# wenyuqing/panacea

Hardware: AMD Instinct MI355X
Metric: denoising steps/s (6-view x 8-frame 256x512) (higher is better)
Workload: dtype f16; 1 GPU; BASELINE config 3: Panacea+ stage-2 UNet+ControlNet, CFG 2 x 8 frames, 6 views, latent 32x384, hint 256x3072, Euler/LegacyDDPM 50-step schedule; precision=precise: split(stream,gn_stt,ff_out,stem,gn_head,gnt)+e4m3-lo, parallelism=single, graph=False, streams=2, hoisted_step_invariants=False, fused_step_tail=True

## Files before the change

### include/panacea_hip.h

```cpp
#ifndef PANACEA_HIP_H
#define PANACEA_HIP_H

#include <stdint.h>

#ifdef __cplusplus
extern "C" {
#endif

#define PNC_OK 0
#define PNC_EINVAL (-1)
#define PNC_EALIGN (-2)
#define PNC_EABI (-3)

const char* pnc_version(void);
#define PNC_ABI_VERSION 8
int pnc_abi_version(void);
const char* pnc_build_digest(void);

enum {
    PNC_OPT_GEMM_TAIL_SPLIT = 0,
    PNC_OPT_GEMM_TILE = 1,
    PNC_OPT_ATTN_VARIANT = 2,
    PNC_OPT_ATTN_DMA = 3,
    PNC_OPT_GEMM_FUSE_LN = 4,
// ... 124 lines not shown
#define PNC_SMALLM_MAX_SEGS 64
int pnc_linear_smallm_segments(const float* a, int lda, const void* W, const float* bias, float* out, int M,
                               int m0, int Mtot, int N, int K, const int32_t* seg_start, int nseg, int silu_in,
                               int silu_out, void* stream);
int pnc_linear_smallm_segments_split(const float* a, int lda, const void* W, const void* W_lo, const float* bias, float* out,
                                     int M, int m0, int Mtot, int N, int K, const int32_t* seg_start, int nseg, int silu_in,
                                     int silu_out, void* stream);
int pnc_timestep_embedding(const int64_t* t, int F, int dim, const float* freqs,
                           float* out, void* stream);
int pnc_timestep_embedding_f32(const float* t, int F, int dim, const float* freqs,
                               float* out, void* stream);
int pnc_nchw_to_tokens_f16(const float* a, int C1, const float* a_scale, int a_frames, const float* b, int C2,
                           int F, int Npix, int Cpad, void* out16, void* out16_lo, void* stream);
int pnc_cfg_euler_step(const float* eps_tok, int ld, int T, int Npix, int C, int cfg, float scale,
                       const float* x, const float* c_out, const float* sigma, const float* sigma_next, float* x_next,
                       void* stream);
enum {
    PNC_SAMPLER_HEUN1 = 0, PNC_SAMPLER_HEUN2 = 1, PNC_SAMPLER_EULER_A = 2, PNC_SAMPLER_DPM2S_1 = 3, PNC_SAMPLER_DPM2S_2 = 4,
    PNC_SAMPLER_DPM2M = 5, PNC_SAMPLER_LMS = 6
};
typedef struct PncSamplerStepParams {
    int32_t struct_bytes;
    int32_t mode;
    const float* eps_tok;
    int32_t ld, T, Npix, C;
    int32_t cfg;
    float scale;
    const float* x;
    const float* c_out;
    const float* x0;
    const float* aux;
    const float* hist[4];
    int32_t n_hist;
    float s_noise;
    const float* noise;
    const float* v[6];
    float* out;
    float* out_aux;
} PncSamplerStepParams;
int pnc_cfg_sampler_step(const PncSamplerStepParams* p, void* stream);
int pnc_cfg_euler_step_skip(const float* eps_tok, int ld, int T, int Npix, int C, int cfg, float scale,
                            const float* x, const float* c_skip, const float* c_out, const float* sigma,
                            const float* sigma_next, float* x_next, void* stream);
int pnc_cfg_sampler_step_skip(const PncSamplerStepParams* p, const float* c_skip, void* stream);
int pnc_tokens_to_nchw_f32(const float* x, int ld, int F, int Npix, int C,
                           float* out, void* stream);
int pnc_concat_add(const float* a, int C1, const float* s, const float* c, int C2,
                   int64_t M, float* out32, void* out16, void* out16_lo, int lo_fmt, void* stream);
int pnc_concat_add_stats(const float* a, int C1, const float* s, const float* c, int C2, int F, int Npix, int pix_per_chunk,
                         float* out32, void* out16, void* out16_lo, int lo_fmt, float* partial, void* stream);
int pnc_add_f32(const float* x, const float* a, int64_t n, float* y32, void* y16, void* y16_lo, int lo_fmt,
                void* stream);
int pnc_cast_f16(const float* x, int64_t n, void* y16, void* y16_lo, int lo_fmt, void* stream);

int pnc_range_monitor_collect(unsigned int* out, void* stream);

#define PNC_STATS_WORDS 36
int pnc_operand_stats_f16(const void* hi, const void* lo, int lo_fmt, int64_t rows, int cols, int64_t ld,
                          unsigned long long* rec, void* stream);

int pnc_softmax_rows_f16(const float* s, int64_t lds, int M, int N, float scale, int causal, int n_valid,
                         void* p16, int64_t ldp, void* stream);

int pnc_attn_frame_f16(const void* q, int64_t ldq, const void* k, int64_t ldk,
                       const void* vt, int64_t ldvt, int64_t vt_fstride,
                       void* o, int64_t ldo, int F, int N, int C, float scale, void* stream);

int pnc_attn_frame_split_f16(const void* q, const void* q_lo, int64_t ldq, const void* k, const void* k_lo, int64_t ldk,
                             const void* v, const void* v_lo, int64_t ldv, void* o, void* o_lo, int64_t ldo,
                             int F, int N, int C, float scale, void* stream);

int pnc_attn_text_split_f16(const void* q, const void* q_lo, int64_t ldq, const void* k, const void* k_lo, int64_t ldk,
                            const void* v, const void* v_lo, int64_t ldv, void* o, void* o_lo, int64_t ldo,
                            int groups, int heads, int Lp, int kv_valid, float scale, void* stream);

int pnc_u8_to_tokens_f16(const uint8_t* src, const float* lut, int F, int Npix, int C, int Cpad,
                         void* out16, void* out16_lo, void* stream);
int pnc_tokens_to_u8(const float* x, int ld, int64_t M, int C, uint8_t* out, void* stream);

#ifdef __cplusplus
}
#endif
#endif
```

### panacea_amd/csrc/misc.hip

```cpp
#include "common.h"
#include <atomic>

namespace {

constexpr int SM_MAXM = 16;

__global__ __launch_bounds__(256) void linear_smallm_kernel(const float* __restrict__ a, int lda,
                                                            const half_t* __restrict__ W,
                                                            const half_t* __restrict__ W_lo,
                                                            const float* __restrict__ bias,
                                                            float* __restrict__ out, int ldo, int M, int N,
                                                            int K, int silu_in, int silu_out) {
    const int lane = threadIdx.x & 63;
    const int n = blockIdx.x * 4 + (threadIdx.x >> 6);
    if (n >= N) return;
    float acc[SM_MAXM];
#pragma unroll
    for (int m = 0; m < SM_MAXM; ++m) acc[m] = 0.0f;
    for (int k0 = lane * 8; k0 < K; k0 += 64 * 8) {
        const half8v w = *reinterpret_cast<const half8v*>(W + (int64_t)n * K + k0);
        float wf[8];
#pragma unroll
        for (int e = 0; e < 8; ++e) wf[e] = (float)w[e];
        if (W_lo) {
// ... 140 lines not shown
                                                             int Npix, int C, float* __restrict__ out) {
    const int64_t i = (int64_t)blockIdx.x * 256 + threadIdx.x;
    if (i >= (int64_t)F * Npix) return;
    const int64_t f = i / Npix, pix = i - f * Npix;
    for (int c = 0; c < C; ++c) out[(f * C + c) * Npix + pix] = x[i * ld + c];
}

__global__ __launch_bounds__(256) void concat_add_kernel(const float* __restrict__ a, int C1,
                                                         const float* __restrict__ s,
                                                         const float* __restrict__ c, int C2, int64_t M,
                                                         float* __restrict__ out32, half_t* __restrict__ out16,
                                                         void* __restrict__ out16_lo, int lo_fmt) {
    const int CT = C1 + C2, V = CT >> 2;
    const int64_t i = (int64_t)blockIdx.x * 256 + threadIdx.x;
    if (i >= M * V) return;
    const int64_t m = i / V;
    const int ch = (int)(i - m * V) * 4;
    f32x4 v;
    if (ch < C1) {
        v = *reinterpret_cast<const f32x4*>(a + m * C1 + ch);
    } else {
        const int c2 = ch - C1;
        v = *reinterpret_cast<const f32x4*>(s + m * C2 + c2);
        if (c) {
            const f32x4 w = *reinterpret_cast<const f32x4*>(c + m * C2 + c2);
            v += w;
        }
    }
    if (out32) *reinterpret_cast<f32x4*>(out32 + m * CT + ch) = v;
    if (out16) {
        half4v h = {(half_t)v[0], (half_t)v[1], (half_t)v[2], (half_t)v[3]};
        *reinterpret_cast<half4v*>(out16 + m * CT + ch) = h;
        if (out16_lo) {
            const float o[4] = {v[0], v[1], v[2], v[3]};
            store_lo4(out16_lo, lo_fmt, m * CT + ch, o, h);
        }
    }
}

__global__ __launch_bounds__(256) void add_kernel(const float* __restrict__ x, const float* __restrict__ a,
                                                  int64_t n4, float* __restrict__ y32, half_t* __restrict__ y16,
                                                  void* __restrict__ y16_lo, int lo_fmt) {
    const int64_t i = (int64_t)blockIdx.x * 256 + threadIdx.x;
    if (i >= n4) return;
    f32x4 v = *reinterpret_cast<const f32x4*>(x + i * 4);
    if (a) { const f32x4 w = *reinterpret_cast<const f32x4*>(a + i * 4); v += w; }
    if (y32) *reinterpret_cast<f32x4*>(y32 + i * 4) = v;
    if (y16) {
        half4v h = {(half_t)v[0], (half_t)v[1], (half_t)v[2], (half_t)v[3]};
        *reinterpret_cast<half4v*>(y16 + i * 4) = h;
        if (y16_lo) {
            const float o[4] = {v[0], v[1], v[2], v[3]};
            store_lo4(y16_lo, lo_fmt, i * 4, o, h);
        }
    }
}

template <bool SKIP>
__device__ __forceinline__ float guided_denoised(float xv, float eu, float ec, float co, float cs, int cfg, float scale) {
#pragma clang fp contract(off)
    const float xs = SKIP ? xv * cs : xv;
    const float pc = ec * co;
    float D = pc + xs;
    if (cfg) {
        const float pu = eu * co;
        const float du = pu + xs;
        const float g = scale * (D - du);
        D = du + g;
    }
    return D;
}

template <bool SKIP>
__global__ __launch_bounds__(256) void cfg_sampler_step_kernel(const PncSamplerStepParams p, const float* __restrict__ c_skip) {
#pragma clang fp contract(off)
    const int64_t i = (int64_t)blockIdx.x * 256 + threadIdx.x;
    if (i >= (int64_t)p.T * p.Npix) return;
    const int64_t t = i / p.Npix, pix = i - t * p.Npix;
    const float co = p.c_out[t];
    const float cs = SKIP ? c_skip[t] : 1.0f;
    const float v0 = p.v[0] ? p.v[0][t] : 0.f, v1 = p.v[1] ? p.v[1][t] : 0.f, v2 = p.v[2] ? p.v[2][t] : 0.f;
    const float v3 = p.v[3] ? p.v[3][t] : 0.f, v4 = p.v[4] ? p.v[4][t] : 0.f;
    const float* eu = p.eps_tok + i * p.ld;
    const float* ec = p.eps_tok + ((int64_t)(p.cfg ? p.T : 0) * p.Npix + i) * p.ld;
    for (int c = 0; c < p.C; ++c) {
        const int64_t o = (t * p.C + c) * p.Npix + pix;
        const float xv = p.x[o];
        const float D = guided_denoised<SKIP>(xv, eu[c], ec[c], co, cs, p.cfg, p.scale);
        float y;
        switch (p.mode) {
        case PNC_SAMPLER_HEUN1: {
            const float d = (xv - D) / v0;
            const float dt = v1 - v0;
            const float stp = dt * d;
            y = xv + stp;
            if (p.out_aux) p.out_aux[o] = d;
            break;
        }
        case PNC_SAMPLER_HEUN2: {
            const float d_new = (xv - D) / v1;
            const float sum = p.aux[o] + d_new;
            const float dp = sum / 2.0f;
            const float dt = v1 - v0;
            const float stp = dp * dt;
            const float xc = p.x0[o] + stp;
            y = v1 > 0.f ? xc : xv;
// ... 178 lines not shown
        segs.start[i] = seg_start[i];
    }
    return launch_1d(linear_smallm_seg_kernel, (int64_t)(N / SEG_NC) * 64, stream, a, lda, f16p(W), f16p(W_lo), bias, out, M, m0, Mtot,
                     N, K, silu_in, silu_out, segs);
}

template <typename TS>
static int timestep_embedding(const TS* t, int F, int dim, const float* freqs, float* out, void* stream) {
    if (!t || !out || !freqs || F < 1 || dim < 2) return PNC_EINVAL;
    return launch_1d(timestep_embedding_kernel<TS>, F * (dim / 2), stream, t, F, dim, freqs, out);
}

extern "C" int pnc_timestep_embedding(const int64_t* t, int F, int dim, const float* freqs,
                                      float* out, void* stream) {
    return timestep_embedding(t, F, dim, freqs, out, stream);
}

extern "C" int pnc_timestep_embedding_f32(const float* t, int F, int dim, const float* freqs,
                                          float* out, void* stream) {
    return timestep_embedding(t, F, dim, freqs, out, stream);
}

extern "C" int pnc_nchw_to_tokens_f16(const float* a, int C1, const float* a_scale, int a_frames, const float* b, int C2,
                                      int F, int Npix, int Cpad, void* out16, void* out16_lo, void* stream) {
    if (!a || !out16 || F < 1 || Npix < 1 || C1 < 1 || C2 < 0 || (C2 > 0 && !b)) return PNC_EINVAL;
    if (a_frames < 1 || a_frames > F) return PNC_EINVAL;
    if (Cpad % 8 || Cpad < C1 + C2) return PNC_EINVAL;
    if (((uintptr_t)out16 | (uintptr_t)out16_lo) & 15) return PNC_EALIGN;
    return launch_1d(nchw_to_tokens_kernel, (int64_t)F * Npix, stream, a, C1, a_scale, a_frames, b, C2, F, Npix, Cpad, f16p(out16),
                     f16p(out16_lo));
}

extern "C" int pnc_tokens_to_nchw_f32(const float* x, int ld, int F, int Npix, int C,
                                      float* out, void* stream) {
    if (!x || !out || F < 1 || Npix < 1 || C < 1 || ld < C) return PNC_EINVAL;
    return launch_1d(tokens_to_nchw_kernel, (int64_t)F * Npix, stream, x, ld, F, Npix, C, out);
}

extern "C" int pnc_concat_add(const float* a, int C1, const float* s, const float* c, int C2,
                              int64_t M, float* out32, void* out16, void* out16_lo, int lo_fmt, void* stream) {
    if (!a || !s || M < 1 || C1 % 4 || C2 % 4 || C1 < 4 || C2 < 4) return PNC_EINVAL;
    if (lo_fmt != PNC_LO_F16 && lo_fmt != PNC_LO_E4M3) return PNC_EINVAL;
    if ((!out32 && !out16) || (out16_lo && !out16)) return PNC_EINVAL;
    return launch_1d(concat_add_kernel, M * ((C1 + C2) / 4), stream, a, C1, s, c, C2, M, out32, f16p(out16), out16_lo, lo_fmt);
}

extern "C" int pnc_add_f32(const float* x, const float* a, int64_t n, float* y32, void* y16, void* y16_lo, int lo_fmt,
                           void* stream) {
    if (!x || n < 4 || n % 4 || (!y32 && !y16) || (y16_lo && !y16)) return PNC_EINVAL;
    if (lo_fmt != PNC_LO_F16 && lo_fmt != PNC_LO_E4M3) return PNC_EINVAL;
    return launch_1d(add_kernel, n / 4, stream, x, a, n / 4, y32, f16p(y16), y16_lo, lo_fmt);
}

__global__ __launch_bounds__(256) void softmax_rows_kernel(const float* __restrict__ s, int64_t lds, int N, float scale,
                                                           int causal, int n_valid,
                                                           half_t* __restrict__ p, int64_t ldp) {
    __shared__ float red[8];
    const int tid = threadIdx.x, lane = tid & 63, wave = tid >> 6;
    const float* row = s + (int64_t)blockIdx.x * lds;
    half_t* prow = p + (int64_t)blockIdx.x * ldp;
    const int nv = N >> 2;
    const int lim = causal ? min(n_valid, (int)blockIdx.x + 1) : n_valid;
    f32x4 v[16];
    float m = -3.0e38f;
#pragma unroll
    for (int j = 0; j < 16; ++j) {
        const int c = tid + j * 256;
        if (c < nv) {
            v[j] = *reinterpret_cast<const f32x4*>(row + c * 4);
#pragma unroll
            for (int e = 0; e < 4; ++e) v[j][e] = (c * 4 + e < lim) ? v[j][e] : -3.0e38f;
            m = fmaxf(fmaxf(fmaxf(v[j][0], v[j][1]), fmaxf(v[j][2], v[j][3])), m);
        }
    }
#pragma unroll
    for (int o = 32; o > 0; o >>= 1) m = fmaxf(m, __shfl_xor(m, o, 64));
    if (lane == 0) red[wave] = m;
    __syncthreads();
    m = fmaxf(fmaxf(red[0], red[1]), fmaxf(red[2], red[3]));
    const float sc = scale * 1.44269504088896340736f;
    const float off = m * sc;
    float sum = 0.0f;
#pragma unroll
    for (int j = 0; j < 16; ++j) {
        const int c = tid + j * 256;
        if (c < nv) {
#pragma unroll
            for (int e = 0; e < 4; ++e) {
                const float pe = __builtin_amdgcn_exp2f(fmaf(v[j][e], sc, -off));
                v[j][e] = (c * 4 + e < lim) ? pe : 0.0f;
                sum += v[j][e];
            }
        }
    }
    sum = wave_sum(sum);
    if (lane == 0) red[4 + wave] = sum;
    __syncthreads();
    const float inv = 1.0f / (((red[4] + red[5]) + red[6]) + red[7]);
#pragma unroll
    for (int j = 0; j < 16; ++j) {
        const int c = tid + j * 256;
        if (c < nv) {
            half4v h;
#pragma unroll
            for (int e = 0; e < 4; ++e) h[e] = (half_t)(v[j][e] * inv);
            *reinterpret_cast<half4v*>(prow + c * 4) = h;
// ... 32 lines not shown
```

### panacea_amd/engine.py

```python
from __future__ import annotations

import contextlib
import dataclasses
import math
import os
from dataclasses import dataclass
from typing import Callable, Dict, List, NamedTuple, Optional

import torch

from . import hip as _hip
from .shard import FrameShard, ViewShard

_BACKEND = _hip


def backend():
    return _BACKEND


@contextlib.contextmanager
def use_backend(be):
    global _BACKEND
    old, _BACKEND = _BACKEND, be
# ... 213 lines not shown
            raise ValueError(f"at most {TEXT_PAD} context tokens are supported, got {n}")
        if D % 8:
            raise ValueError("context_dim must be a multiple of 8")
        self.n_text = n
        if self.prec.ctx:
            c32 = torch.zeros((B, TEXT_PAD, D), device=self.device, dtype=torch.float32)
            c32[:, :n] = context.to(device=self.device, dtype=torch.float32)
            self.ctx16 = self.operand((B * TEXT_PAD, D), "ctx")
            self.be.cast_f16(c32, c32.numel(), *self.ctx16)
            return
        c = torch.zeros((B, TEXT_PAD, D), device=self.device, dtype=torch.float16)
        c[:, :n] = context.to(device=self.device, dtype=torch.float16)
        self.ctx16 = Operand(c.view(B * TEXT_PAD, D))
        if self.profile is not None:
            self.profile.note(c, "ctx")


def _f16_from_bits(bits: int) -> float:
    import struct
    return struct.unpack("<e", struct.pack("<H", int(bits) & 0xFFFF))[0]


class RangeProfile:
    WORDS = _hip.STATS_WORDS

    def __init__(self, device, slots: int = 4096):
        self.table = torch.zeros((slots, self.WORDS), dtype=torch.int64, device=device)
        self.sites: List[tuple] = []
        self.evaluations = 0
        self.limit: Optional[int] = None
        self._slot: Dict[tuple, int] = {}
        self._cls: Dict[int, str] = {}
        self._names: Dict[int, str] = {}

    def bind(self, network: torch.nn.Module):
        for name, m in network.named_modules():
            self._names.setdefault(id(m), name)

    def note(self, t: torch.Tensor, cls: Optional[str]):
        ptr = t.untyped_storage().data_ptr()
        if cls is None:
            self._cls.pop(ptr, None)
        else:
            self._cls[ptr] = cls

    def begin_evaluation(self):
        self._cls.clear()
        self.evaluations += 1

    def class_of(self, t: torch.Tensor) -> str:
        return self._cls.get(t.untyped_storage().data_ptr(), "unsplit")

    def _site(self, pk, key, site) -> str:
        if key is None:
            owner, name = site if site is not None else (None, "stacked")
        else:
            owner, name = getattr(pk, "owner", None), ".".join(str(k) for k in (key if isinstance(key, tuple) else (key,)))
        mod = "" if owner is None else self._names.get(id(owner), type(owner).__name__)
        return f"{mod}.{name}" if mod else name

    def observe(self, rt: Runtime, a: Operand, pk, key, site, kw: dict):
        if rt.shard is not None or rt.vshard is not None:
            raise ValueError("the range profile does not run frame- or view-sharded")
        mode = kw.get("a_mode", _hip.A_PLAIN)
        if mode == _hip.A_PLAIN:
            rows, cols = kw["M"], kw["K"]
            ld = kw.get("lda") or cols
        elif mode == _hip.A_CONV3X3:
            c = kw["conv"]
            cols = ld = c["Cin"]
            rows = kw["M"] // (c["Hout"] * c["Wout"]) * c["Hin"] * c["Win"]
        else:
            cols = ld = kw["tconv"]["C"]
            rows = kw["M"]
        k = (self.class_of(a.hi), self._site(pk, key, site))
        slot = self._slot.get(k)
        if slot is None:
            if len(self.sites) >= self.table.shape[0]:
                raise ValueError(f"the range profile holds {self.table.shape[0]} sites; make it with more slots")
            slot = self._slot[k] = len(self.sites)
            self.sites.append(k)
        rt.be.operand_stats(a.hi, a.lo, rows, cols, ld, self.table[slot])

    @staticmethod
    def _stats(words, max_bits: int) -> dict:
        b = [int(v) for v in words[:32]]
        return {"elements": int(words[35]), "max_abs": _f16_from_bits(max_bits), "binades": b, "ge_512": sum(b[24:]),
                "lo_saturated": int(words[33]), "nan": int(words[34]), "inf": b[31] - int(words[34])}

    def report(self) -> dict:
        n = len(self.sites)
        host = self.table[:n].cpu().tolist() if n else []
        order = sorted(range(n), key=lambda i: (-host[i][32], self.sites[i][1], self.sites[i][0]))
        sites = [{"site": self.sites[i][1], "class": self.sites[i][0], **self._stats(host[i], host[i][32])} for i in order]
        sums: Dict[str, list] = {}
        for (cls, _), w in zip(self.sites, host):
            s = sums.setdefault(cls, [0] * self.WORDS)
            for j in range(self.WORDS):
                s[j] = max(s[j], w[j]) if j == 32 else s[j] + w[j]
        return {"evaluations": self.evaluations, "classes": {c: self._stats(w, w[32]) for c, w in sorted(sums.items())}, "sites": sites}

    def recommend(self, network: torch.nn.Module) -> dict:
        rep = self.report()
        split = [c for c in OPERAND_CLASSES if getattr(PRECISE, c) and c in rep["classes"]]
        top = max((b for c in split for b, cnt in enumerate(rep["classes"][c]["binades"]) if cnt), default=0)
        headroom = 24 - top
        s = rep["sites"][0] if rep["sites"] else None
# ... 17 lines not shown


def split_lo(w: torch.Tensor, hi16: torch.Tensor) -> torch.Tensor:
    return ((w.detach().to(torch.float32) - hi16.to(torch.float32)) * 2048.0).to(torch.float16)


def _cast16(w: torch.Tensor, lo: bool = False) -> torch.Tensor:
    w = w.detach()
    hi = w.to(torch.float16)
    return split_lo(w, hi) if lo else hi


def lo_planes(packed):
    if isinstance(packed, torch.Tensor):
        return packed if packed.dtype == torch.float16 else None
    if isinstance(packed, dict):
        return {k: lo_planes(v) for k, v in packed.items()}
    if isinstance(packed, (list, tuple)):
        return type(packed)(lo_planes(v) for v in packed)
    return packed


def pk_f16(w: torch.Tensor, lo: bool = False) -> torch.Tensor:
    return _cast16(w, lo).contiguous()


def pk_f32(w: Optional[torch.Tensor]) -> Optional[torch.Tensor]:
    return None if w is None else w.detach().to(torch.float32).contiguous()


def pk_linear(w: torch.Tensor, lo: bool = False) -> torch.Tensor:
    return pk_f16(w.reshape(w.shape[0], -1), lo)


def pk_lo8(w16: torch.Tensor):
    w = w16.detach().float()
    amax = float(w.abs().max())
    sh = 0 if amax == 0.0 else int(math.floor(math.log2(448.0 / amax)))
    sh = max(-126, min(126, sh))
    q = (w * (2.0 ** sh)).clamp_(-448.0, 448.0).to(torch.float8_e4m3fn)
    return q.view(torch.uint8).contiguous(), 127 - sh


def pk_conv3x3(w: torch.Tensor, cin_pad: Optional[int] = None, lo: bool = False) -> torch.Tensor:
    co, ci = w.shape[0], w.shape[1]
    cp = cin_pad or ((ci + 7) // 8 * 8)
    p = torch.zeros((co, 3, 3, cp), device=w.device, dtype=torch.float16)
    p[..., :ci] = _cast16(w.detach().permute(0, 2, 3, 1), lo)
    if cp % 64 == 0:
        p = p.view(co, 9, cp // 64, 64).permute(0, 2, 1, 3)
    return p.reshape(co, 9 * cp).contiguous()


def pk_conv1d(w: torch.Tensor, lo: bool = False) -> torch.Tensor:
    co, ci = w.shape[0], w.shape[1]
    p = w.detach().permute(0, 2, 1)
    if ci % 64 == 0:
        p = p.reshape(co, 3, ci // 64, 64).permute(0, 2, 1, 3)
    return pk_f16(p.reshape(co, -1), lo)


def pk_geglu(w: torch.Tensor, b: torch.Tensor, lo: bool = False):
    n2 = w.shape[0] // 2
    if n2 % 32:
        raise ValueError("GEGLU inner dim must be a multiple of 32")
    wv, wg = w[:n2].view(n2 // 32, 32, -1), w[n2:].view(n2 // 32, 32, -1)
    wi = torch.stack([wv, wg], dim=1).reshape(2 * n2, -1)
    bi = torch.stack([b[:n2].view(-1, 32), b[n2:].view(-1, 32)], dim=1).reshape(-1)
    return pk_f16(wi, lo), pk_f32(bi)


PERM16 = (0, 1, 2, 3, 8, 9, 10, 11, 4, 5, 6, 7, 12, 13, 14, 15)


def mfma_a_fragments(w16: torch.Tensor) -> torch.Tensor:
    R, S = w16.shape[0] // 32, w16.shape[1] // 16
    wp = w16.reshape(R, 32, S, 16)[..., list(PERM16)]
    return wp.reshape(R, 32, S, 2, 8).permute(0, 2, 3, 1, 4).reshape(R, S, 64, 8).contiguous()


class Packed(dict):
    owner = None

    def lo(self) -> dict:
        return self.owner.packed_lo()


class Packable:
    _pk: Optional[dict] = None
    _pk_lo: Optional[dict] = None

    def _init_packable(self):
        self._pk = None
        self._pk_lo = None
        self.register_load_state_dict_post_hook(lambda m, _k: m.invalidate_packed())

    def invalidate_packed(self):
        self._pk = None
        self._pk_lo = None

    def _apply(self, fn, *a, **k):
        self.invalidate_packed()
        return super()._apply(fn, *a, **k)

    def packed(self) -> dict:
        if self._pk is None:
            with torch.no_grad():
                self._pk = Packed(self._pack())
                self._pk.owner = self
        return self._pk

    def packed_lo(self) -> dict:
        if self._pk_lo is None:
            with torch.no_grad():
                self._pk_lo = lo_planes(self._pack(lo=True))
        return self._pk_lo

    def _pack(self, lo: bool = False) -> dict:
        raise NotImplementedError


def invalidate_all(module: torch.nn.Module):
    for m in module.modules():
        if isinstance(m, Packable):
            m.invalidate_packed()


def _ppc(npix: int) -> int:
    return max(16, min(128, npix // 48), -(-npix // 256))


GN_EPILOGUE_CHUNK = 64
GN_FROM_EPILOGUE = True
EMB_BATCH = os.environ.get("PNC_EMB_BATCH", "1") != "0"
TEXTKV_ONE_GEMM = os.environ.get("PNC_TEXTKV_ONE_GEMM", "1") != "0"


def gn_records(rt: Runtime, F: int, N: int) -> Optional[torch.Tensor]:
    if not GN_FROM_EPILOGUE:
        return None
    return rt.empty((F * (-(-N // GN_EPILOGUE_CHUNK)) * 32 * 3,), torch.float32)


def gn_spatial(rt: Runtime, x32: torch.Tensor, F: int, N: int, C: int, gamma, beta, eps: float, silu: bool,
               split: Optional[str] = None, tail_rows: int = 0, part: Optional[torch.Tensor] = None):
    if C % 64:
        raise ValueError(f"GroupNorm(32) kernels need C % 64 == 0, got {C}")
    ppc = _ppc(N)
    y, ylo = out = rt.operand((F * N, C), split, tail_rows)
    if part is None:
        nrec = (N + ppc - 1) // ppc
        part = rt.empty((F * nrec * 32 * 3,), torch.float32)
        rt.be.groupnorm_stats(x32, C, F, N, C, ppc, part)
    else:
        nrec = part.numel() // (F * 96)
    vs = rt.vshard
    if vs is not None and tail_rows and vs.fused_halo and tail_rows % (2 * F) == 0 and N % (tail_rows // (2 * F)) == 0:
        H = tail_rows // (2 * F)
        W = N // H
        x4 = x32.view(F, H, W, C)
        allp, fl, fr = vs.stats_and_halo(part, x4[:, :, 0], x4[:, :, W - 1], F, nrec)
        comb = torch.empty((F * nrec * 96,), device=x32.device, dtype=torch.float32)
        rt.be.groupnorm_combine(allp, vs.G if vs.group is not None else 1, F, nrec, comb)
        rt.be.groupnorm_apply(x32, C, F, N, C, ppc, comb, gamma, beta, eps, silu, y, C, ylo, n_records=nrec)
        for side, raw in ((0, fl), (1, fr)):
            for pl in (y, ylo):
                if pl is None:
                    continue
                t = pl._pnc_tail[F * N + side * F * H: F * N + (side + 1) * F * H]
                if raw is None:
                    t.zero_()
            if raw is not None:
                yt = y._pnc_tail[F * N + side * F * H: F * N + (side + 1) * F * H]
                lt = None if ylo is None else ylo._pnc_tail[F * N + side * F * H: F * N + (side + 1) * F * H]
                rt.be.groupnorm_apply(raw.reshape(F * H, C).contiguous(), C, F, H, C, ppc, comb, gamma, beta, eps, silu, yt, C, lt,
                                      n_records=nrec)
        for pl in out.planes():
            pl._pnc_halo_ready = True
        return out
    if vs is not None:
        part = vs.combine_stats(part, F, nrec, rt.be)
    rt.be.groupnorm_apply(x32, C, F, N, C, ppc, part, gamma, beta, eps, silu, y, C, ylo, n_records=nrec)
    return out


def gn_temporal(rt: Runtime, x32: torch.Tensor, N: int, C: int, gamma, beta, eps: float) -> Operand:
    y = rt.operand((rt.B * rt.T * N, C), "gnt")
    rt.be.groupnorm_temporal_silu(x32, rt.B, rt.T, N, C, gamma, beta, eps, *y)
# ... 111 lines not shown
```

### panacea_amd/hip.py

```python
from __future__ import annotations

import ctypes as C
import re
from pathlib import Path
from typing import Optional

import torch

PKG = Path(__file__).resolve().parent
LIB_PATH = PKG / "lib" / "libpanacea_hip.so"
HEADER = PKG.parent / "include" / "panacea_hip.h"

A_PLAIN, A_CONV3X3, A_CONV1D_T = 0, 1, 2
ACT_NONE, ACT_SILU, ACT_GELU = 0, 1, 2
ABI_VERSION = 8
LO_F16, LO_E4M3 = 0, 1
LO_DTYPE = {LO_F16: torch.float16, LO_E4M3: torch.uint8}


def lo_fmt(t: Optional[torch.Tensor]) -> int:
    if t is None or t.dtype == torch.float16:
        return LO_F16
    if t.dtype == torch.uint8:
        return LO_E4M3
# ... 64 lines not shown
        ("struct_bytes", C.c_int32), ("mode", C.c_int32),
        ("eps_tok", C.c_void_p), ("ld", C.c_int32), ("T", C.c_int32), ("Npix", C.c_int32), ("C", C.c_int32),
        ("cfg", C.c_int32), ("scale", C.c_float),
        ("x", C.c_void_p), ("c_out", C.c_void_p), ("x0", C.c_void_p), ("aux", C.c_void_p),
        ("hist", C.c_void_p * 4), ("n_hist", C.c_int32), ("s_noise", C.c_float), ("noise", C.c_void_p),
        ("v", C.c_void_p * 6), ("out", C.c_void_p), ("out_aux", C.c_void_p),
    ]


SAMPLER_HEUN1, SAMPLER_HEUN2, SAMPLER_EULER_A, SAMPLER_DPM2S_1, SAMPLER_DPM2S_2, SAMPLER_DPM2M, SAMPLER_LMS = range(7)


_P, _I, _L, _F = C.c_void_p, C.c_int, C.c_int64, C.c_float
_SIGNATURES = {
    "pnc_version": (C.c_char_p, []),
    "pnc_abi_version": (_I, []),
    "pnc_build_digest": (C.c_char_p, []),
    "pnc_set_option": (_I, [_I, _I]),
    "pnc_gemm_f16": (_I, [C.POINTER(GemmParams), _P]),
    "pnc_gemm_wsplit_f16": (_I, [C.POINTER(GemmParams), _P, _P]),
    "pnc_gemm_workspace_floats": (_L, [C.POINTER(GemmParams)]),
    "pnc_gemm_fuses_layernorm": (_I, [C.POINTER(GemmParams)]),
    "pnc_attn_views_f16": (_I, [C.POINTER(AttnParams), _P]),
    "pnc_attn_uses_text_kernel": (_I, [C.POINTER(AttnParams)]),
    "pnc_attn_views_split_f16": (_I, [C.POINTER(AttnSplitParams), _P]),
    "pnc_attn_temporal_split_f16": (_I, [_P, _P, _I, _P, _P, _I, _P, _P, _I, _P, _P, _I, _I, _I, _I, _I, _F, _P]),
    "pnc_softmax_rows_f16": (_I, [_P, _L, _I, _I, _F, _I, _I, _P, _L, _P]),
    "pnc_attn_temporal_f16": (_I, [_P, _I, _P, _I, _P, _I, _P, _I, _I, _I, _I, _I, _F, _P]),
    "pnc_attn_frame_f16": (_I, [_P, _L, _P, _L, _P, _L, _L, _P, _L, _I, _I, _I, _F, _P]),
    "pnc_attn_frame_split_f16": (_I, [_P, _P, _L, _P, _P, _L, _P, _P, _L, _P, _P, _L, _I, _I, _I, _F, _P]),
    "pnc_attn_text_split_f16": (_I, [_P, _P, _L, _P, _P, _L, _P, _P, _L, _P, _P, _L, _I, _I, _I, _I, _F, _P]),
    "pnc_groupnorm_stats": (_I, [_P, _I, _I, _I, _I, _I, _P, _P]),
    "pnc_groupnorm_apply": (_I, [_P, _I, _I, _I, _I, _I, _P, _P, _P, _F, _I, _P, _I, _P, _I, _I, _P]),
    "pnc_groupnorm_combine": (_I, [_P, _I, _I, _I, _P, _P]),
    "pnc_groupnorm_temporal_part": (_I, [_P, _I, _I, _I, _I, _P, _P, _F, _P, _I, _I, _P, _P, _I, _I, _P]),
    "pnc_groupnorm_temporal_silu": (_I, [_P, _I, _I, _I, _I, _P, _P, _F, _P, _P, _I, _P]),
    "pnc_layernorm": (_I, [_P, _I, _I, _I, _P, _P, _F, _P, _I, _P, _P]),
    "pnc_linear_smallm": (_I, [_P, _I, _P, _P, _P, _I, _I, _I, _I, _I, _I, _P]),
    "pnc_linear_smallm_segments": (_I, [_P, _I, _P, _P, _P, _I, _I, _I, _I, _I, _P, _I, _I, _I, _P]),
    "pnc_linear_smallm_split": (_I, [_P, _I, _P, _P, _P, _P, _I, _I, _I, _I, _I, _I, _P]),
    "pnc_linear_smallm_segments_split": (_I, [_P, _I, _P, _P, _P, _P, _I, _I, _I, _I, _I, _P, _I, _I, _I, _P]),
    "pnc_timestep_embedding": (_I, [_P, _I, _I, _P, _P, _P]),
    "pnc_timestep_embedding_f32": (_I, [_P, _I, _I, _P, _P, _P]),
    "pnc_nchw_to_tokens_f16": (_I, [_P, _I, _P, _I, _P, _I, _I, _I, _I, _P, _P, _P]),
    "pnc_cfg_euler_step": (_I, [_P, _I, _I, _I, _I, _I, _F, _P, _P, _P, _P, _P, _P]),
    "pnc_cfg_sampler_step": (_I, [C.POINTER(SamplerStepParams), _P]),
    "pnc_cfg_euler_step_skip": (_I, [_P, _I, _I, _I, _I, _I, _F, _P, _P, _P, _P, _P, _P, _P]),
    "pnc_cfg_sampler_step_skip": (_I, [C.POINTER(SamplerStepParams), _P, _P]),
    "pnc_tokens_to_nchw_f32": (_I, [_P, _I, _I, _I, _I, _P, _P]),
    "pnc_concat_add": (_I, [_P, _I, _P, _P, _I, _L, _P, _P, _P, _I, _P]),
    "pnc_concat_add_stats": (_I, [_P, _I, _P, _P, _I, _I, _I, _I, _P, _P, _P, _I, _P, _P]),
    "pnc_add_f32": (_I, [_P, _P, _L, _P, _P, _P, _I, _P]),
    "pnc_cast_f16": (_I, [_P, _L, _P, _P, _I, _P]),
    "pnc_range_monitor_collect": (_I, [_P, _P]),
    "pnc_operand_stats_f16": (_I, [_P, _P, _I, _L, _I, _L, _P, _P]),
    "pnc_u8_to_tokens_f16": (_I, [_P, _P, _I, _I, _I, _I, _P, _P, _P]),
    "pnc_tokens_to_u8": (_I, [_P, _I, _L, _I, _P, _P]),
}

_lib = None


def header_symbols() -> list[str]:
    txt = HEADER.read_text()
    txt = re.sub(r"/\*.*?\*/", "", txt, flags=re.S)
    return sorted(set(re.findall(r"\b(pnc_[a-z0-9_]+)\s*\(", txt)))


def load():
    global _lib
    if _lib is not None:
        return _lib
    import os
    global LIB_PATH
    if os.environ.get("PANACEA_HIP_LIB"):
        LIB_PATH = Path(os.environ["PANACEA_HIP_LIB"])
    if not LIB_PATH.exists():
        raise HipLibraryError(
            f"{LIB_PATH} is missing: the HIP extension is the only compute path of panacea_amd. "
            "Build it with `python -m panacea_amd.build` (hipcc --offload-arch=gfx950).")
    try:
        lib = C.CDLL(str(LIB_PATH))
    except OSError as e:
        raise HipLibraryError(f"cannot load {LIB_PATH}: {e}") from e
    if not os.environ.get("PANACEA_HIP_LIB"):
        from . import build as _build
        try:
            lib.pnc_build_digest.restype = C.c_char_p
            have = lib.pnc_build_digest().decode()
        except AttributeError:
            have = "(a library older than pnc_build_digest)"
        if _build.CSRC.exists() and have != _build._digest():
            raise HipLibraryError(f"{LIB_PATH} was built from other sources ({have[:12]}) than panacea_amd/csrc holds now "
                                  f"({_build._digest()[:12]}); rebuild it with `python -m panacea_amd.build`")
    for name, (res, args) in _SIGNATURES.items():
        try:
            fn = getattr(lib, name)
        except AttributeError as e:
            raise HipLibraryError(f"{LIB_PATH} does not export {name}; rebuild the extension") from e
        fn.restype = res
        fn.argtypes = args
    if lib.pnc_abi_version() != ABI_VERSION:
        raise HipLibraryError(f"{LIB_PATH} implements C-ABI version {lib.pnc_abi_version()}, this binding needs "
                              f"{ABI_VERSION}; rebuild the extension (`python -m panacea_amd.build --force`)")
    _lib = lib
    return lib
# ... 376 lines not shown
        raise PncError(f"tokens_to_u8: out is {M} x {Cch} contiguous bytes, got {tuple(out_u8.shape)}")
    _check(_timed("layout", 0.0, M * Cch * 5.0, load().pnc_tokens_to_u8, _ptr(x32, torch.float32, "x"), ld, M, Cch,
                  _ptr(out_u8, torch.uint8, "out"), _stream()), "pnc_tokens_to_u8")


def cfg_euler_step(eps_tok, ld, T, Npix, Cch, cfg, scale, x, c_out, sigma, sigma_next, x_next, c_skip=None):
    name, skip = _sibling("pnc_cfg_euler_step", "_skip", c_skip, "c_skip", torch.float32)
    _check(_timed("elementwise", 0.0, T * Npix * Cch * (16.0 if cfg else 12.0), getattr(load(), name), _ptr(eps_tok), ld, T, Npix, Cch,
                  int(cfg), float(scale), _ptr(x), *skip, _ptr(c_out), _ptr(sigma), _ptr(sigma_next), _ptr(x_next), _stream()), name)


def cfg_sampler_step(mode, eps_tok, ld, T, Npix, Cch, cfg, scale, x, c_out, v, out, out_aux=None, x0=None, aux=None,
                     hist=(), noise=None, s_noise=1.0, c_skip=None):
    p = SamplerStepParams()
    p.struct_bytes = C.sizeof(SamplerStepParams)
    f32 = torch.float32
    p.mode, p.ld, p.T, p.Npix, p.C, p.cfg, p.scale = mode, ld, T, Npix, Cch, int(cfg), float(scale)
    p.eps_tok, p.x, p.c_out = _ptr(eps_tok, f32, "eps_tok"), _ptr(x, f32, "x"), _ptr(c_out, f32, "c_out")
    p.x0, p.aux, p.noise = _ptr(x0, f32, "x0"), _ptr(aux, f32, "aux"), _ptr(noise, f32, "noise")
    p.out, p.out_aux = _ptr(out, f32, "out"), _ptr(out_aux, f32, "out_aux")
    if len(v) > 6 or len(hist) > 4:
        raise PncError("cfg_sampler_step: at most 6 per-frame vectors and 4 history planes")
    for k, t in enumerate(v):
        p.v[k] = _ptr(t, f32, f"v[{k}]")
    for k, t in enumerate(hist):
        p.hist[k] = _ptr(t, f32, f"hist[{k}]")
    p.n_hist, p.s_noise = len(hist), float(s_noise)
    planes = 3 + (x0 is not None) + (aux is not None) + (noise is not None) + (out_aux is not None) + len(hist)
    nbytes = T * Npix * Cch * (4.0 * planes + (4.0 if cfg else 0.0))
    name, skip = _sibling("pnc_cfg_sampler_step", "_skip", c_skip, "c_skip", f32)
    _check(_timed("elementwise", 0.0, nbytes, getattr(load(), name), C.byref(p), *skip, _stream()), name)


def tokens_to_nchw_f32(x32, ld, F, Npix, Cch, out32):
    _check(load().pnc_tokens_to_nchw_f32(_ptr(x32), ld, F, Npix, Cch, _ptr(out32), _stream()),
           "pnc_tokens_to_nchw_f32")


def concat_add(a32, C1, s32, c32, C2, M, out32, out16, out16_lo=None, gn_part=None, frames=0, ppc=64):
    nb = M * (4.0 * C1 + (8.0 if c32 is not None else 4.0) * C2 + (6.0 + _lo_bytes(out16_lo)) * (C1 + C2))
    if gn_part is not None and (frames < 1 or M % frames):
        raise PncError(f"concat_add with gn_part: M = {M} rows are not {frames} whole frames")
    name, part = _sibling("pnc_concat_add", "_stats", gn_part, "gn_part", torch.float32)
    rows = (frames, M // frames, ppc) if part else (M,)
    _check(_timed("elementwise", 0.0, nb, getattr(load(), name), _ptr(a32), C1, _ptr(s32), _ptr(c32), C2, *rows, _ptr(out32), _ptr(out16),
                  _ptr(out16_lo), lo_fmt(out16_lo), *part, _stream()), name)


def add_f32(x32, a32, n, y32, y16, y16_lo=None):
    _check(_timed("elementwise", 0.0, 12.0 * n, load().pnc_add_f32, _ptr(x32), _ptr(a32), n, _ptr(y32), _ptr(y16),
                  _ptr(y16_lo), lo_fmt(y16_lo), _stream()), "pnc_add_f32")


def range_monitor_collect(out_i32: torch.Tensor):
    _check(load().pnc_range_monitor_collect(_ptr(out_i32, torch.int32, "out"), _stream()), "pnc_range_monitor_collect")


STATS_WORDS = 36


def operand_stats(hi, lo, rows, cols, ld, rec):
    if rec.dtype != torch.int64 or rec.numel() < STATS_WORDS or not rec.is_contiguous():
        raise PncError(f"operand_stats: the record is {STATS_WORDS} contiguous int64 words, got {rec.dtype} x {rec.numel()}")
    fmt = lo_fmt(lo)
    nb = rows * cols * (2.0 + _lo_bytes(lo))
    _check(_timed("operand_stats", 0.0, nb, load().pnc_operand_stats_f16, _ptr(hi, torch.float16, "hi"), _ptr(lo, LO_DTYPE[fmt], "lo"),
                  fmt, rows, cols, ld, _ptr(rec, torch.int64, "rec"), _stream()), "pnc_operand_stats_f16")


def cast_f16(x32, n, y16, y16_lo=None):
    _check(load().pnc_cast_f16(_ptr(x32), n, _ptr(y16), _ptr(y16_lo), lo_fmt(y16_lo), _stream()), "pnc_cast_f16")
```

### panacea_amd/nn/openaimodel.py

```python
from __future__ import annotations

import contextlib
from typing import Optional

import torch
import torch.nn as nn

from .. import engine as E
from ..engine import Act, Packable, Runtime
from .attention import SpatialTemporalTransformer
from .util import check_num_frames, conv_nd, linear, normalization, timestep_embedding, zero_module


def _as_list(v):
    if isinstance(v, (int, float)) or v is None:
        return v
    return list(v)


class TimestepBlock(nn.Module):
    """openaimodel.py:66-76 — marker for children that take the timestep embedding."""


def conv_params(conv: nn.Conv2d, lo=False):
# ... 21 lines not shown
    o16 = rt.operand((M, Cout), split_out) if out16 else None
    E.gemm(rt, x, pk, key, o16, M=M, N=Cout, K=9 * Cin_pad, a_mode=E._hip.A_CONV3X3, conv=conv, bias=bias,
           act=E._hip.ACT_SILU if act_silu else E._hip.ACT_NONE, out32=o32, ldc32=Cout, ldc16=Cout)
    return Act(F, Hout, Wout, Cout, f32=o32, f16=o16)


class TimestepEmbedSequential(nn.Sequential, TimestepBlock, Packable):

    def __init__(self, *args):
        super().__init__(*args)
        self._init_packable()

    def _pack(self, lo=False):
        return {i: conv_params(m, lo) for i, m in enumerate(self) if isinstance(m, nn.Conv2d)}

    def _run(self, rt: Runtime, x: Act, emb32, want_f16: bool = False) -> Act:
        layers = list(self)
        for i, layer in enumerate(layers):
            nxt = layers[i + 1] if i + 1 < len(layers) else None
            wf = want_f16 if nxt is None else isinstance(nxt, (Upsample, Downsample, nn.Conv2d))
            if isinstance(layer, ResBlock3D):
                x = layer._run(rt, x, emb32, want_f16=wf, want_stats=isinstance(nxt, (ResBlock3D, SpatialTemporalTransformer)))
            elif isinstance(layer, SpatialTemporalTransformer):
                x = layer._run(rt, x, want_f16=wf)
            elif isinstance(layer, (Upsample, Downsample)):
                x = layer._run(rt, x, want_f16=wf)
            elif isinstance(layer, nn.Conv2d):
                pk, Co = self.packed(), layer.out_channels
                if layer.kernel_size[0] == 3:
                    x = run_conv3x3(rt, x.need_f16(rt), x.F, x.H, x.W, x.C, pk, i, Co, stride=layer.stride[0], out16=wf,
                                    split_out="stream")
                else:
                    o32 = rt.empty((x.M, Co), torch.float32)
                    o16 = rt.operand((x.M, Co), "stream") if wf else None
                    E.gemm(rt, x.need_f16(rt), pk, i, o16, M=x.M, N=Co, K=x.C, lda=x.C, out32=o32, ldc32=Co, ldc16=Co)
                    x = Act(x.F, x.H, x.W, Co, f32=o32, f16=o16)
            else:
                raise NotImplementedError(f"{type(layer).__name__} inside TimestepEmbedSequential")
        return x


class Upsample(nn.Module, Packable):

    def __init__(self, channels, use_conv, dims=2, out_channels=None, padding=1, third_up=False):
        super().__init__()
        if dims != 2 or not use_conv or padding != 1:
            raise NotImplementedError("Upsample: only dims=2 with a 3x3 conv is on the Panacea path")
        self.channels, self.out_channels, self.use_conv, self.dims = channels, out_channels or channels, use_conv, dims
        self.conv = conv_nd(dims, self.channels, self.out_channels, 3, padding=padding)
        self._init_packable()

    def _pack(self, lo=False):
        w, b = conv_params(self.conv, lo)
        return dict(w=w, b=b)

    precise_operand = True

    def _run(self, rt: Runtime, x: Act, want_f16=False) -> Act:
        pk = self.packed()
        x16 = x.need_f16(rt)
        if not self.precise_operand:
            x16 = E.Operand(x16.hi)
        return run_conv3x3(rt, x16, x.F, x.H, x.W, x.C, pk, "w", self.out_channels, pk["b"], upsample=True, out16=want_f16,
                           split_out="stream")


class Downsample(nn.Module, Packable):

    def __init__(self, channels, use_conv, dims=2, out_channels=None, padding=1, third_down=False):
        super().__init__()
        if dims != 2 or not use_conv or padding != 1:
            raise NotImplementedError("Downsample: only dims=2 with a strided 3x3 conv is on the Panacea path")
        self.channels, self.out_channels, self.use_conv, self.dims = channels, out_channels or channels, use_conv, dims
        self.op = conv_nd(dims, self.channels, self.out_channels, 3, stride=2, padding=padding)
        self._init_packable()

    def _pack(self, lo=False):
        w, b = conv_params(self.op, lo)
        return dict(w=w, b=b)

    def _run(self, rt: Runtime, x: Act, want_f16=False) -> Act:
        pk = self.packed()
        return run_conv3x3(rt, x.need_f16(rt), x.F, x.H, x.W, x.C, pk, "w", self.out_channels, pk["b"], stride=2, out16=want_f16,
                           split_out="stream")


class ResBlock3D(TimestepBlock, Packable):

    def __init__(self, channels, emb_channels, dropout, out_channels=None, use_conv=False,
                 use_scale_shift_norm=False, dims=2, use_checkpoint=False, up=False, down=False, kernel_size=3,
                 exchange_temb_dims=False, skip_t_emb=False, temporal_kernel_size=3, alpha=1, num_frames=4):
        super().__init__()
        if up or down or use_scale_shift_norm or exchange_temb_dims or skip_t_emb or use_conv:
            raise NotImplementedError("ResBlock3D: up/down/scale-shift/exchange_temb/skip_t_emb/use_conv are dead "
                                      "paths of the Panacea configuration and are not built")
        if dims != 2 or kernel_size != 3 or temporal_kernel_size != 3:
            raise NotImplementedError("ResBlock3D: dims=2, 3x3 spatial and k=3 temporal kernels only")
        self.num_frames = check_num_frames(num_frames, "ResBlock3D")
        self.channels, self.emb_channels, self.dropout = channels, emb_channels, dropout
        self.out_channels = out_channels or channels
        self.use_conv, self.use_checkpoint, self.use_scale_shift_norm = use_conv, use_checkpoint, use_scale_shift_norm
        self.exchange_temb_dims = exchange_temb_dims
        self.alpha = 1 if alpha == 1 else nn.Parameter(torch.rand(1, requires_grad=True))
        self.temporal_kernel_size = temporal_kernel_size
        self.identity_layer = nn.Identity()
        oc = self.out_channels
        self.in_layers = nn.Sequential(normalization(channels), nn.SiLU(), conv_nd(dims, channels, oc, 3, padding=1))
        self.in_layers_temporal = nn.Sequential(normalization(oc), nn.SiLU(),
                                                zero_module(conv_nd(1, oc, oc, 3, padding=1)))
        self.updown = False
        self.h_upd = self.x_upd = nn.Identity()
        self.skip_t_emb = skip_t_emb
        self.emb_out_channels = oc
        self.emb_layers = nn.Sequential(nn.SiLU(), linear(emb_channels, oc))
        self.out_layers = nn.Sequential(normalization(oc), nn.SiLU(), nn.Dropout(p=dropout),
                                        zero_module(conv_nd(dims, oc, oc, 3, padding=1)))
        self.out_layers_temporal = nn.Sequential(normalization(oc), nn.SiLU(), nn.Dropout(p=dropout),
# ... 560 lines not shown
```

Baseline: 6.392 steps/s.

## Compute upsample conv at source resolution via per-tap GEMM and combine kernel

Replaces the nearest-upsample-then-3x3-conv path with one GEMM at the input resolution. The GEMM yields all 9 tap products per pixel, and a new combine kernel sums the overlapping taps for each of the four output sub-pixels, adding the bias and writing f32/f16/lo outputs. Since nearest upsampling repeats pixels, this cuts the GEMM M dimension by a factor of four. In exchange it writes and reads a large 9*Cout f32 intermediate, chunked by frames, and changes the order of summation.

```diff
diff --git a/include/panacea_hip.h b/include/panacea_hip.h
--- a/include/panacea_hip.h
+++ b/include/panacea_hip.h
@@ -200,6 +200,8 @@
 int pnc_add_f32(const float* x, const float* a, int64_t n, float* y32, void* y16, void* y16_lo, int lo_fmt,
                 void* stream);
 int pnc_cast_f16(const float* x, int64_t n, void* y16, void* y16_lo, int lo_fmt, void* stream);
+int pnc_upsample_combine(const float* P, int64_t ldp, const float* bias, int F, int Hin, int Win, int Cout, float* out32,
+                         void* out16, void* out16_lo, int lo_fmt, void* stream);
 
 int pnc_range_monitor_collect(unsigned int* out, void* stream);
 
diff --git a/panacea_amd/csrc/misc.hip b/panacea_amd/csrc/misc.hip
--- a/panacea_amd/csrc/misc.hip
+++ b/panacea_amd/csrc/misc.hip
@@ -216,6 +216,71 @@
         if (y16_lo) {
             const float o[4] = {v[0], v[1], v[2], v[3]};
             store_lo4(y16_lo, lo_fmt, i * 4, o, h);
+        }
+    }
+}
+
+constexpr int UC_TQ = 32, UC_TW = 4, UC_TH = 2;
+static_assert(UC_TQ * UC_TW * UC_TH == 256, "one work item per thread of the 256-thread workgroup");
+
+__global__ __launch_bounds__(256) void upsample_combine_kernel(const float* __restrict__ P, int64_t ldp,
+                                                               const float* __restrict__ bias, int Hin, int Win, int Cout,
+                                                               int tiles_x, int tiles_y, int qslices,
+                                                               float* __restrict__ out32, half_t* __restrict__ out16,
+                                                               void* __restrict__ out16_lo, int lo_fmt) {
+    int b = xcd_remap((int)blockIdx.x, (int)gridDim.x);
+    const int tx = b % tiles_x; b /= tiles_x;
+    const int ty = b % tiles_y; b /= tiles_y;
+    const int qs = b % qslices;
+    const int f = b / qslices;
+    const int tid = threadIdx.x;
+    const int q = qs * UC_TQ + (tid & (UC_TQ - 1));
+    const int pix = tid / UC_TQ;
+    const int sx = tx * UC_TW + (pix % UC_TW), sy = ty * UC_TH + (pix / UC_TW);
+    if (q * 4 >= Cout || sx >= Win || sy >= Hin) return;
+    const int n = q * 4;
+    constexpr int SU[5] = {0, 0, 1, 2, 2}, SD[5] = {-1, 0, 0, 0, 1};
+    constexpr int SEL[2][3] = {{0, 2, 3}, {1, 2, 4}};
+    const bool rv[5] = {sy > 0, true, true, true, sy + 1 < Hin};
+    const bool cv[5] = {sx > 0, true, true, true, sx + 1 < Win};
+    const float* Pn = P + n;
+    f32x4 v[5][5];
+#pragma unroll
+    for (int i = 0; i < 5; ++i) {
+#pragma unroll
+        for (int j = 0; j < 5; ++j) {
+            if (rv[i] && cv[j]) {
+                const int64_t row = ((int64_t)f * Hin + (sy + SD[i])) * Win + (sx + SD[j]);
+                v[i][j] = *reinterpret_cast<const f32x4*>(Pn + row * ldp + (int64_t)(SU[i] * 3 + SU[j]) * Cout);
+            } else {
+                v[i][j] = f32x4{0.0f, 0.0f, 0.0f, 0.0f};
+            }
+        }
+    }
+    const f32x4 bv = bias ? *reinterpret_cast<const f32x4*>(bias + n) : f32x4{0.0f, 0.0f, 0.0f, 0.0f};
+#pragma unroll
+    for (int dy = 0; dy < 2; ++dy) {
+#pragma unroll
+        for (int dx = 0; dx < 2; ++dx) {
+            f32x4 acc = bv;
+#pragma unroll
+            for (int u = 0; u < 3; ++u) {
+#pragma unroll
+                for (int w = 0; w < 3; ++w) {
+                    const int i = SEL[dy][u], j = SEL[dx][w];
+                    if (rv[i] && cv[j]) acc += v[i][j];
+                }
+            }
+            const int64_t o = (((int64_t)f * (2 * Hin) + (2 * sy + dy)) * (2 * Win) + (2 * sx + dx)) * Cout + n;
+            *reinterpret_cast<f32x4*>(out32 + o) = acc;
+            if (out16) {
+                half4v h = {(half_t)acc[0], (half_t)acc[1], (half_t)acc[2], (half_t)acc[3]};
+                *reinterpret_cast<half4v*>(out16 + o) = h;
+                if (out16_lo) {
+                    const float r[4] = {acc[0], acc[1], acc[2], acc[3]};
+                    store_lo4(out16_lo, lo_fmt, o, r, h);
+                }
+            }
         }
     }
 }
@@ -500,6 +565,19 @@
     return launch_1d(add_kernel, n / 4, stream, x, a, n / 4, y32, f16p(y16), y16_lo, lo_fmt);
 }
 
+extern "C" int pnc_upsample_combine(const float* P, int64_t ldp, const float* bias, int F, int Hin, int Win, int Cout, float* out32,
+                                    void* out16, void* out16_lo, int lo_fmt, void* stream) {
+    if (!P || !out32 || F < 1 || Hin < 1 || Win < 1 || Cout < 4 || Cout % 4 || ldp % 4 || ldp < 9 * (int64_t)Cout) return PNC_EINVAL;
+    if (lo_fmt != PNC_LO_F16 && lo_fmt != PNC_LO_E4M3) return PNC_EINVAL;
+    if (out16_lo && !out16) return PNC_EINVAL;
+    if (((uintptr_t)P | (uintptr_t)bias | (uintptr_t)out32 | (uintptr_t)out16 | (uintptr_t)out16_lo) & 15) return PNC_EALIGN;
+    const int tiles_x = (Win + UC_TW - 1) / UC_TW, tiles_y = (Hin + UC_TH - 1) / UC_TH, qslices = (Cout / 4 + UC_TQ - 1) / UC_TQ;
+    const int64_t blocks = (int64_t)F * tiles_y * tiles_x * qslices;
+    if (blocks >= ((int64_t)1 << 31)) return PNC_EINVAL;
+    return launch_1d(upsample_combine_kernel, blocks * 256, stream, P, ldp, bias, Hin, Win, Cout, tiles_x, tiles_y, qslices, out32,
+                     f16p(out16), out16_lo, lo_fmt);
+}
+
 __global__ __launch_bounds__(256) void softmax_rows_kernel(const float* __restrict__ s, int64_t lds, int N, float scale,
                                                            int causal, int n_valid,
                                                            half_t* __restrict__ p, int64_t ldp) {
diff --git a/panacea_amd/engine.py b/panacea_amd/engine.py
--- a/panacea_amd/engine.py
+++ b/panacea_amd/engine.py
@@ -289,7 +289,7 @@
         return self._cls.get(t.untyped_storage().data_ptr(), "unsplit")
 
     def _site(self, pk, key, site) -> str:
-        if key is None:
+        if key is None or site is not None:
             owner, name = site if site is not None else (None, "stacked")
         else:
             owner, name = getattr(pk, "owner", None), ".".join(str(k) for k in (key if isinstance(key, tuple) else (key,)))
@@ -413,6 +413,10 @@
     return p.reshape(co, 9 * cp).contiguous()
 
 
+def pk_conv3x3_taps(w: torch.Tensor, lo: bool = False) -> torch.Tensor:
+    return pk_linear(w.detach().permute(2, 3, 0, 1).reshape(9 * w.shape[0], w.shape[1]), lo)
+
+
 def pk_conv1d(w: torch.Tensor, lo: bool = False) -> torch.Tensor:
     co, ci = w.shape[0], w.shape[1]
     p = w.detach().permute(0, 2, 1)
@@ -495,6 +499,14 @@
 GN_FROM_EPILOGUE = True
 EMB_BATCH = os.environ.get("PNC_EMB_BATCH", "1") != "0"
 TEXTKV_ONE_GEMM = os.environ.get("PNC_TEXTKV_ONE_GEMM", "1") != "0"
+UPSAMPLE_SOURCE_RES = os.environ.get("PNC_UPSAMPLE_SOURCE_RES", "1") != "0"
+UPSAMPLE_CHUNK_FRAMES = int(os.environ.get("PNC_UPSAMPLE_CHUNK_FRAMES", "0"))
+
+
+def upsample_chunk_frames(F: int, Hin: int, Win: int, Cout: int) -> int:
+    if UPSAMPLE_CHUNK_FRAMES > 0:
+        return min(F, UPSAMPLE_CHUNK_FRAMES)
+    return max(1, min(F, (1 << 31) // (36 * Cout * Hin * Win)))
 
 
 def gn_records(rt: Runtime, F: int, N: int) -> Optional[torch.Tensor]:
diff --git a/panacea_amd/hip.py b/panacea_amd/hip.py
--- a/panacea_amd/hip.py
+++ b/panacea_amd/hip.py
@@ -140,6 +140,7 @@
     "pnc_concat_add_stats": (_I, [_P, _I, _P, _P, _I, _I, _I, _I, _P, _P, _P, _I, _P, _P]),
     "pnc_add_f32": (_I, [_P, _P, _L, _P, _P, _P, _I, _P]),
     "pnc_cast_f16": (_I, [_P, _L, _P, _P, _I, _P]),
+    "pnc_upsample_combine": (_I, [_P, _L, _P, _I, _I, _I, _I, _P, _P, _P, _I, _P]),
     "pnc_range_monitor_collect": (_I, [_P, _P]),
     "pnc_operand_stats_f16": (_I, [_P, _P, _I, _L, _I, _L, _P, _P]),
     "pnc_u8_to_tokens_f16": (_I, [_P, _P, _I, _I, _I, _I, _P, _P, _P]),
@@ -622,6 +623,19 @@
                   _ptr(y16_lo), lo_fmt(y16_lo), _stream()), "pnc_add_f32")
 
 
+def upsample_combine(P, ldp, bias, F, Hin, Win, Cout, out32, out16=None, out16_lo=None):
+    rows, outs = F * Hin * Win, 4 * F * Hin * Win * Cout
+    short = [t for t in (out32, out16, out16_lo) if t is not None and t.numel() < outs]
+    if P.numel() < (rows - 1) * ldp + 9 * Cout or short:
+        raise PncError(f"upsample_combine: P holds {rows} rows of {9 * Cout} products (ldp {ldp}) and every output {outs} elements")
+    fmt = lo_fmt(out16_lo)
+    nb = 36.0 * rows * Cout + outs * (4.0 + (2.0 if out16 is not None else 0.0) + _lo_bytes(out16_lo))
+    _check(_timed("upsample_combine", 0.0, nb, load().pnc_upsample_combine, _ptr(P, torch.float32, "P"), ldp,
+                  _ptr(bias, torch.float32, "bias"), F, Hin, Win, Cout, _ptr(out32, torch.float32, "out32"),
+                  _ptr(out16, torch.float16, "out16"), _ptr(out16_lo, LO_DTYPE[fmt], "out16_lo"), fmt, _stream()),
+           "pnc_upsample_combine")
+
+
 def range_monitor_collect(out_i32: torch.Tensor):
     _check(load().pnc_range_monitor_collect(_ptr(out_i32, torch.int32, "out"), _stream()), "pnc_range_monitor_collect")
 
diff --git a/panacea_amd/nn/openaimodel.py b/panacea_amd/nn/openaimodel.py
--- a/panacea_amd/nn/openaimodel.py
+++ b/panacea_amd/nn/openaimodel.py
@@ -97,7 +97,7 @@
 
     def _pack(self, lo=False):
         w, b = conv_params(self.conv, lo)
-        return dict(w=w, b=b)
+        return dict(w=w, b=b, w9=E.pk_conv3x3_taps(self.conv.weight, lo))
 
     precise_operand = True
 
@@ -106,8 +106,22 @@
         x16 = x.need_f16(rt)
         if not self.precise_operand:
             x16 = E.Operand(x16.hi)
-        return run_conv3x3(rt, x16, x.F, x.H, x.W, x.C, pk, "w", self.out_channels, pk["b"], upsample=True, out16=want_f16,
-                           split_out="stream")
+        Co = self.out_channels
+        combine = getattr(rt.be, "upsample_combine", None)
+        if not (E.UPSAMPLE_SOURCE_RES and combine is not None and rt.vshard is None and x.C % 64 == 0 and Co % 4 == 0):
+            return run_conv3x3(rt, x16, x.F, x.H, x.W, x.C, pk, "w", Co, pk["b"], upsample=True, out16=want_f16, split_out="stream")
+        N, Mo = x.N, 4 * x.M
+        o32 = rt.empty((Mo, Co), torch.float32)
+        o16 = rt.operand((Mo, Co), "stream") if want_f16 else None
+        fc = E.upsample_chunk_frames(x.F, x.H, x.W, Co)
+        P = rt.empty((fc * N, 9 * Co), torch.float32)
+        for f0 in range(0, x.F, fc):
+            nf = min(fc, x.F - f0)
+            E.gemm(rt, x16.map(lambda t: t[f0 * N:(f0 + nf) * N]), pk, "w9", site=(self, "w"), M=nf * N, N=9 * Co, K=x.C, lda=x.C,
+                   out32=P, ldc32=9 * Co)
+            outs = [None if t is None else t[4 * f0 * N:] for t in (o32, *(o16 or (None, None)))]
+            combine(P, 9 * Co, pk["b"], nf, x.H, x.W, Co, *outs)
+        return Act(x.F, 2 * x.H, 2 * x.W, Co, f32=o32, f16=o16)
 
 
 class Downsample(nn.Module, Packable):
```

Measured after the change: 6.511 steps/s (median of 6 runs). 1.02x the previous value.
